# WangHelin1997/SSR-Speech

Hardware: AMD Instinct MI355X
Metric: codec-tokens/sec/GPU (AR decode) + RTF for 10 s TTS, English 830M (higher is better)
Workload: dtype f32; 1 GPU; English-830M-shape zero-shot TTS decode, cfg_stride=5, top_k=40/top_p=0.8 sampling, batch=1 (2 CFG rows) per GPU; L=130 phonemes, 160-frame prompt (demo/5895_34622_000026_000002.wav, first 3.2 s, wmencodec codes), context 304..324; utterances_per_gpu=1, rows=2, graph=True, steps_completed=25, pair_launches=True

## Files before the change

ssr-speech_amd/csrc/embed_sample.hip:

```cpp
#include <stdlib.h>
#include "common.h"

namespace {

__device__ __forceinline__ void embed_row(const ssrhip_embed_args& a, int r, int kind, int pos, const int* tok, int t0, int nt) {
  const int D = a.D;
  const float alpha = kind ? a.alpha_audio : a.alpha_text;
  for (int d = t0 * 4; d < D; d += nt * 4) {
    float4 e;
    if (kind == 0) {
      e = ld4(a.text_emb + (size_t)tok[0] * D + d);
    } else {
      float4 t[SSRHIP_MAX_CODEBOOKS];
#pragma unroll
      for (int k = 0; k < SSRHIP_MAX_CODEBOOKS; ++k)
        t[k] = (k < a.K) ? ld4(a.audio_emb + ((size_t)k * a.card + tok[k]) * D + d) : make_float4(0.f, 0.f, 0.f, 0.f);
      e = t[0];
#pragma unroll
      for (int k = 1; k < SSRHIP_MAX_CODEBOOKS; ++k) {
        if (k < a.K) { e.x += t[k].x; e.y += t[k].y; e.z += t[k].z; e.w += t[k].w; }
      }
    }
    const float4 p = ld4(a.pe + (size_t)pos * D + d);
    e.x = __fadd_rn(e.x, __fmul_rn(alpha, p.x));
    e.y = __fadd_rn(e.y, __fmul_rn(alpha, p.y));
    e.z = __fadd_rn(e.z, __fmul_rn(alpha, p.z));
    e.w = __fadd_rn(e.w, __fmul_rn(alpha, p.w));
    float* dst = a.out_tiled ? a.out + SSRHIP_TILED_P(r, d, D) : a.out + (size_t)r * D + d;
    *reinterpret_cast<float4*>(dst) = e;
  }
}

__global__ __launch_bounds__(256) void embed_kernel(const ssrhip_embed_args a) {
  const int r = blockIdx.x;
  embed_row(a, r, a.kind ? a.kind[r] : 1, a.pos[r], a.tok + (size_t)r * SSRHIP_MAX_CODEBOOKS, threadIdx.x, 256);
}

constexpr int MAXE = 9;
constexpr int WPC = 4;
constexpr int SAMPLE_THREADS = 64 * WPC * SSRHIP_MAX_CODEBOOKS;

#ifdef SSR_SAMPLE_PROFILE
__device__ unsigned long long g_sample_prof[16];
#define STAMP(i) do { if (threadIdx.x == 0) g_sample_prof[i] = __builtin_readcyclecounter(); } while (0)
#else
#define STAMP(i) do { } while (0)
#endif

__device__ __forceinline__ uint32_t okey(float f) {
  const uint32_t u = __float_as_uint(f);
  return (u & 0x80000000u) ? ~u : (u | 0x80000000u);
}

__device__ __forceinline__ uint32_t hash32(uint32_t x) {
  x ^= x >> 16; x *= 0x7feb352du; x ^= x >> 15; x *= 0x846ca68bu; x ^= x >> 16;
  return x;
}

template <class T>
__device__ __forceinline__ T suffix_excl(T v, int lane) {
  T inc = v;
#pragma unroll
  for (int o = 1; o < 64; o <<= 1) {
    const T t = __shfl_down(inc, o, 64);
    if (lane + o < 64) inc += t;
  }
  return inc - v;
}

struct SelShared {
  unsigned long long hist[SSRHIP_MAX_CODEBOOKS][WPC][256];
  unsigned long long carry[SSRHIP_MAX_CODEBOOKS];
  unsigned bin[SSRHIP_MAX_CODEBOOKS];
  int found[SSRHIP_MAX_CODEBOOKS];
  static constexpr int MAXC = 64;
  unsigned ckey[SSRHIP_MAX_CODEBOOKS][MAXC];
  unsigned long long cmass[SSRHIP_MAX_CODEBOOKS][MAXC];
  int ncand[SSRHIP_MAX_CODEBOOKS];
  unsigned result[SSRHIP_MAX_CODEBOOKS];
  int overflow;
};

template <int MODE>
__device__ __forceinline__ uint32_t radix_select(const uint32_t (&key)[MAXE], const float (&p)[MAXE], unsigned kk, float lim, bool active,
                                                 SelShared& sh, int k, int sub, int lane) {
  const float SC = 1099511627776.0f;
  const unsigned long long limfx = (unsigned long long)((double)lim * (double)SC);
  uint32_t prefix = 0, mask = 0;
  unsigned long long carry = (MODE == 0) ? (unsigned long long)kk : 0ull;
  bool keep_all = false;
  for (int pass = 0; pass < 4; ++pass) {
    const int shift = 24 - 8 * pass;
    unsigned long long* mine64 = sh.hist[k][sub];
    unsigned* mine32 = reinterpret_cast<unsigned*>(mine64);
    if (MODE == 0) { for (int j = lane; j < 256; j += 64) mine32[j] = 0u; }
    else { for (int j = lane; j < 256; j += 64) mine64[j] = 0ull; }
    __syncthreads();
    if (active && !keep_all) {
#pragma unroll
      for (int e = 0; e < MAXE; ++e) {
        const bool in = (MODE == 0) ? (key[e] != 0u) : (p[e] > 0.f);
        if (in && (key[e] & mask) == prefix) {
          if (MODE == 0) atomicAdd(&mine32[(key[e] >> shift) & 255u], 1u);
          else atomicAdd(&mine64[(key[e] >> shift) & 255u], (unsigned long long)(p[e] * SC));
        }
      }
    }
    __syncthreads();
    if (sub == 0 && active && !keep_all) {
      unsigned long long c[4] = {0ull, 0ull, 0ull, 0ull};
#pragma unroll
      for (int w = 0; w < WPC; ++w)
#pragma unroll
        for (int j = 0; j < 4; ++j)
          c[j] += (MODE == 0) ? (unsigned long long)reinterpret_cast<unsigned*>(sh.hist[k][w])[lane * 4 + j] : sh.hist[k][w][lane * 4 + j];
      const unsigned long long base = (MODE == 0) ? 0ull : carry;
      const unsigned long long a3 = base + suffix_excl<unsigned long long>(c[0] + c[1] + c[2] + c[3], lane);
      const unsigned long long a2 = a3 + c[3], a1 = a2 + c[2], a0 = a1 + c[1];
      int f = -1;
      unsigned long long above = 0;
      if (MODE == 0) {
        if (carry > a3 && carry <= a3 + c[3]) { f = 3; above = a3; }
        else if (carry > a2 && carry <= a2 + c[2]) { f = 2; above = a2; }
        else if (carry > a1 && carry <= a1 + c[1]) { f = 1; above = a1; }
        else if (carry > a0 && carry <= a0 + c[0]) { f = 0; above = a0; }
      } else {
        if (a3 <= limfx && limfx < a3 + c[3]) { f = 3; above = a3; }
        else if (a2 <= limfx && limfx < a2 + c[2]) { f = 2; above = a2; }
        else if (a1 <= limfx && limfx < a1 + c[1]) { f = 1; above = a1; }
        else if (a0 <= limfx && limfx < a0 + c[0]) { f = 0; above = a0; }
      }
      const unsigned long long bal = __ballot(f >= 0);
      if (lane == 0) sh.found[k] = bal ? 1 : 0;
      if (f >= 0) {
        sh.bin[k] = (unsigned)(lane * 4 + f);
        sh.carry[k] = (MODE == 0) ? (carry - above) : above;
      }
    }
    __syncthreads();
    if (active && !keep_all) {
      if (!sh.found[k]) keep_all = true;
      else {
        prefix |= sh.bin[k] << shift;
        mask |= 255u << shift;
        carry = sh.carry[k];
      }
    }
  }
  return keep_all ? 0u : prefix;
}

template <int MODE>
__device__ __forceinline__ uint32_t bin_select(const uint32_t (&key)[MAXE], const float (&p)[MAXE], const float (&l)[MAXE], float lo, float scale,
                                               unsigned kk, float lim, bool active, SelShared& sh, int k, int sub, int lane, int force_radix, bool& fallback) {
  const float SC = 1099511627776.0f;
  const unsigned long long limfx = (unsigned long long)((double)lim * (double)SC);
  unsigned long long* mine64 = sh.hist[k][sub];
  unsigned* mine32 = reinterpret_cast<unsigned*>(mine64);
  if (MODE == 0) { for (int j = lane; j < 256; j += 64) mine32[j] = 0u; }
  else { for (int j = lane; j < 256; j += 64) mine64[j] = 0ull; }
  if (threadIdx.x == 0) sh.overflow = force_radix;
  if (sub == 0 && lane == 0) { sh.ncand[k] = 0; sh.result[k] = 0u; }
  if (MODE == 0) STAMP(9);
  int vb[MAXE];
#pragma unroll
  for (int e = 0; e < MAXE; ++e) {
    const bool in = (MODE == 0) ? (key[e] != 0u) : (p[e] > 0.f);
    const int ob = min(254, max(1, 1 + (int)((l[e] - lo) * scale)));
    vb[e] = !in ? -1 : (l[e] >= 9000.f ? 255 : (l[e] <= -9000.f ? 0 : ob));
  }
  __syncthreads();
  if (MODE == 0) STAMP(10);
  if (active) {
#pragma unroll
    for (int e = 0; e < MAXE; ++e) {
      if (vb[e] >= 0) {
        if (MODE == 0) atomicAdd(&mine32[vb[e]], 1u);
        else atomicAdd(&mine64[vb[e]], (unsigned long long)(p[e] * SC));
      }
    }
  }
  __syncthreads();
  if (MODE == 0) STAMP(11);
  if (sub == 0 && active) {
    unsigned long long c[4] = {0ull, 0ull, 0ull, 0ull};
#pragma unroll
    for (int w = 0; w < WPC; ++w)
#pragma unroll
      for (int j = 0; j < 4; ++j)
        c[j] += (MODE == 0) ? (unsigned long long)reinterpret_cast<unsigned*>(sh.hist[k][w])[lane * 4 + j] : sh.hist[k][w][lane * 4 + j];
    const unsigned long long a3 = suffix_excl<unsigned long long>(c[0] + c[1] + c[2] + c[3], lane);
    const unsigned long long a2 = a3 + c[3], a1 = a2 + c[2], a0 = a1 + c[1];
    const unsigned long long need = (unsigned long long)kk;
    int f = -1;
    unsigned long long above = 0;
    if (MODE == 0) {
      if (need > a3 && need <= a3 + c[3]) { f = 3; above = a3; }
      else if (need > a2 && need <= a2 + c[2]) { f = 2; above = a2; }
      else if (need > a1 && need <= a1 + c[1]) { f = 1; above = a1; }
      else if (need > a0 && need <= a0 + c[0]) { f = 0; above = a0; }
    } else {
      if (a3 <= limfx && limfx < a3 + c[3]) { f = 3; above = a3; }
      else if (a2 <= limfx && limfx < a2 + c[2]) { f = 2; above = a2; }
      else if (a1 <= limfx && limfx < a1 + c[1]) { f = 1; above = a1; }
      else if (a0 <= limfx && limfx < a0 + c[0]) { f = 0; above = a0; }
    }
    const unsigned long long bal = __ballot(f >= 0);
    if (lane == 0) sh.found[k] = bal ? 1 : 0;
    if (f >= 0) {
      sh.bin[k] = (unsigned)(lane * 4 + f);
      sh.carry[k] = above;
    }
  }
  __syncthreads();
  if (MODE == 0) STAMP(12);
  const bool found = active && sh.found[k];
  const int bsel = found ? (int)sh.bin[k] : -2;
  const unsigned long long above_bins = found ? sh.carry[k] : 0ull;
  if (found) {
#pragma unroll
    for (int e = 0; e < MAXE; ++e) {
      if (vb[e] == bsel) {
        const int idx = atomicAdd(&sh.ncand[k], 1);
        if (idx < SelShared::MAXC) {
          sh.ckey[k][idx] = key[e];
          sh.cmass[k][idx] = (MODE == 0) ? 1ull : (unsigned long long)(p[e] * SC);
        }
      }
    }
  }
  __syncthreads();
  if (MODE == 0) STAMP(13);
  const int n = found ? sh.ncand[k] : 0;
  if (n > SelShared::MAXC) sh.overflow = 1;
  __syncthreads();
  if (MODE == 0) STAMP(14);
  fallback = sh.overflow != 0;
  if (!fallback) {
    unsigned todo = 0u;
#pragma unroll
    for (int e = 0; e < MAXE; ++e) todo |= (found && vb[e] == bsel) ? (1u << e) : 0u;
    while (__any(todo != 0u)) {
      uint32_t ke = 0u;
      bool mine = false;
      if (todo) {
        const int e0 = __builtin_ctz(todo);
        todo &= todo - 1u;
        mine = true;
#pragma unroll
        for (int e = 0; e < MAXE; ++e) ke = (e == e0) ? key[e] : ke;
      }
      unsigned long long A = above_bins, M = 0ull;
      for (int i = 0; i < n; ++i) {
        const unsigned ck = sh.ckey[k][i];
        const unsigned long long m = sh.cmass[k][i];
        A += (ck > ke) ? m : 0ull;
        M += (ck == ke) ? m : 0ull;
      }
      const bool hit = (MODE == 0) ? ((unsigned long long)kk > A && (unsigned long long)kk <= A + M) : (A <= limfx && limfx < A + M);
      if (mine && hit) sh.result[k] = ke;
    }
  }
  __syncthreads();
  if (MODE == 0) STAMP(15);
  return (found && !fallback) ? sh.result[k] : 0u;
}

__global__ __launch_bounds__(SAMPLE_THREADS) void sample_kernel(const ssrhip_sample_args a, const int force_radix) {
  __shared__ SelShared sel;
  __shared__ float sh_f[SSRHIP_MAX_CODEBOOKS][WPC];
  __shared__ float sh_g[SSRHIP_MAX_CODEBOOKS][WPC];
  __shared__ int sh_i[SSRHIP_MAX_CODEBOOKS][WPC];
  __shared__ int sh_sample[SSRHIP_MAX_CODEBOOKS];
  __shared__ int sh_argmax0;
  __shared__ int sh_next[SSRHIP_MAX_CODEBOOKS + 2];
  const int u = blockIdx.x;
  const ssrhip_sampler_cfg& c = a.cfg[u];
  ssrhip_sampler_state& st = a.state[u];
  if (st.done) return;
  const int lane = threadIdx.x & 63, wave = threadIdx.x >> 6;
  const int k = wave / WPC, sub = wave % WPC;
  const int K = a.K, card = a.card;
  const bool active = k < K;
  const int rows = c.use_cfg ? 2 : 1;
  const int row0 = u * rows;
  const int num_gen = st.num_gen, num_eog = st.num_eog, cfg_tag = st.num_cfg_tag;
  const int prev_token = st.prev_token, consec = st.consec_silence;
  const int step = st.n_steps;
  const int c_eos = c.eos, c_sos = c.sos, c_mts = c.mts, c_mts_end = c.mts + c.max_n_spans;
  const int c_empty = c.empty_token, c_eog = c.eog, c_topk = c.top_k, c_stoprep = c.stop_repetition;
  const float c_topp = c.top_p, c_temp = c.temperature, c_coef = c.cfg_coef, c_om = c.cfg_one_minus;
  const int c_maxsteps = c.max_steps, c_nsil = c.n_silence;
  const uint32_t c_seedlo = c.seed_lo, c_seedhi = c.seed_hi;
  const int c_usecfg = c.use_cfg, c_stride = c.cfg_stride, c_textlen = c.text_len, c_nspans = c.n_spans;
  const int st_audio_pos = st.audio_pos, st_span = st.span;
  int c_sil[SSRHIP_MAX_SILENCE];
#pragma unroll
  for (int j = 0; j < SSRHIP_MAX_SILENCE; ++j) c_sil[j] = c.silence[j];
  STAMP(0);

  const int kc = active ? k : 0;
  const float* lc = a.logits + ((size_t)row0 * K + kc) * card;
  const float* lu = lc + (size_t)K * card;
  const bool guided = c_usecfg && (cfg_tag == c_stride);
  bool penal = false;
  if (k == 0 && num_eog == 0 && c_stoprep > 0 && consec > c_stoprep) {
#pragma unroll
    for (int s = 0; s < SSRHIP_MAX_SILENCE; ++s) penal |= (s < c_nsil) && (c_sil[s] == prev_token);
  }
  const float npen = (float)(consec - (c_stoprep - 1));
  const bool force_empty = (num_gen < K - 1) && (k > num_gen);
  const bool cut_eog_empty = (num_eog > 0) && (k > num_eog);
  const bool cut_eog = (num_eog == 0) && (k >= 1);
  float l[MAXE], lun[MAXE];
#pragma unroll
  for (int e = 0; e < MAXE; ++e) {
    const int i = e * 256 + sub * 64 + lane;
    const int ic = (i < card) ? i : 0;
    l[e] = lc[ic];
    lun[e] = guided ? lu[ic] : 0.f;
  }
#pragma unroll
  for (int e = 0; e < MAXE; ++e) {
    const int i = e * 256 + sub * 64 + lane;
    float v = guided ? __fadd_rn(__fmul_rn(c_coef, l[e]), __fmul_rn(c_om, lun[e])) : l[e];
    const bool special = (i == c_eos) | (i == c_sos) | ((i >= c_mts) & (i < c_mts_end));
    v = special ? -10000.f : v;
    v = (force_empty & (i == c_empty)) ? 10000.f : v;
    v = (cut_eog_empty & ((i == c_eog) | (i == c_empty))) ? -10000.f : v;
    v = (cut_eog & (i == c_eog)) ? -10000.f : v;
    if (penal && i == prev_token) v = (v < 0.f) ? __fmul_rn(v, npen) : __fdiv_rn(v, npen);
    l[e] = (active && i < card) ? v : -INFINITY;
  }
  if (a.dbg_logits && active) {
    float* dbg = a.dbg_logits + ((size_t)u * K + k) * card;
#pragma unroll
    for (int e = 0; e < MAXE; ++e) {
      const int i = e * 256 + sub * 64 + lane;
      if (i < card) dbg[i] = l[e];
    }
  }
  STAMP(1);
  float mx = -INFINITY;
#pragma unroll
  for (int e = 0; e < MAXE; ++e) mx = fmaxf(mx, l[e]);
  mx = wave_max(mx);
  int am = 0x7fffffff;
#pragma unroll
  for (int e = 0; e < MAXE; ++e) if (l[e] == mx) am = min(am, e * 256 + sub * 64 + lane);
  am = wave_min_i(am);
  if (lane == 0 && active) { sh_f[k][sub] = mx; sh_i[k][sub] = am; }
  __syncthreads();
  if (active) {
    float m2 = sh_f[k][0];
    int a2 = sh_i[k][0];
#pragma unroll
    for (int w = 1; w < WPC; ++w)
      if (sh_f[k][w] > m2 || (sh_f[k][w] == m2 && sh_i[k][w] < a2)) { m2 = sh_f[k][w]; a2 = sh_i[k][w]; }
    mx = m2;
    am = a2;
  }
  __syncthreads();
  if (c_temp != 1.0f) {
#pragma unroll
    for (int e = 0; e < MAXE; ++e) l[e] = __fdiv_rn(l[e], c_temp);
    float m3 = -INFINITY;
#pragma unroll
    for (int e = 0; e < MAXE; ++e) m3 = fmaxf(m3, l[e]);
    m3 = wave_max(m3);
    if (lane == 0 && active) sh_f[k][sub] = m3;
    __syncthreads();
    if (active) mx = fmaxf(fmaxf(sh_f[k][0], sh_f[k][1]), fmaxf(sh_f[k][2], sh_f[k][3]));
    __syncthreads();
  }
  uint32_t key[MAXE];
#pragma unroll
  for (int e = 0; e < MAXE; ++e) key[e] = (active && (e * 256 + sub * 64 + lane) < card) ? okey(l[e]) : 0u;
  const uint32_t kmax = okey(mx);
  float vlo = INFINITY, vhi = -INFINITY;
#pragma unroll
  for (int e = 0; e < MAXE; ++e) {
    const bool ord = (key[e] != 0u) && (l[e] < 9000.f) && (l[e] > -9000.f);
    vlo = ord ? fminf(vlo, l[e]) : vlo;
    vhi = ord ? fmaxf(vhi, l[e]) : vhi;
  }
  vlo = -wave_max(-vlo);
  vhi = wave_max(vhi);
  if (lane == 0 && active) { sh_f[k][sub] = vlo; sh_g[k][sub] = vhi; }
  __syncthreads();
  if (active) {
    vlo = fminf(fminf(sh_f[k][0], sh_f[k][1]), fminf(sh_f[k][2], sh_f[k][3]));
    vhi = fmaxf(fmaxf(sh_g[k][0], sh_g[k][1]), fmaxf(sh_g[k][2], sh_g[k][3]));
  }
  __syncthreads();
  const float vscale = (vhi > vlo) ? 253.0f / (vhi - vlo) : 0.f;
  float p[MAXE];
#pragma unroll
  for (int e = 0; e < MAXE; ++e) p[e] = 0.f;
  STAMP(2);
  uint32_t thr = 0;
  if (c_topk > 0) {
    const int kk = min(max(c_topk, 1), card);
    if (kk == 1) thr = kmax;
    else if (kk < card) {
      bool fb;
      thr = bin_select<0>(key, p, l, vlo, vscale, (unsigned)kk, 0.f, active, sel, kc, sub, lane, force_radix, fb);
      if (fb) thr = radix_select<0>(key, p, (unsigned)kk, 0.f, active, sel, kc, sub, lane);
    }
  }
  STAMP(3);
  float Z = 0.f;
#pragma unroll
  for (int e = 0; e < MAXE; ++e) {
    p[e] = (key[e] != 0u && key[e] >= thr) ? __expf(l[e] - mx) : 0.f;
    Z += p[e];
  }
  Z = wave_sum(Z);
  if (lane == 0 && active) sh_f[k][sub] = Z;
  __syncthreads();
  if (active) Z = (sh_f[k][0] + sh_f[k][1]) + (sh_f[k][2] + sh_f[k][3]);
  __syncthreads();
  if (c_topp < 1.0f) {
    bool fb;
    uint32_t tp = bin_select<1>(key, p, l, vlo, vscale, 0u, c_topp * Z, active, sel, kc, sub, lane, force_radix, fb);
    if (fb) tp = radix_select<1>(key, p, 0u, c_topp * Z, active, sel, kc, sub, lane);
    if (tp > thr) {
      thr = tp;
#pragma unroll
      for (int e = 0; e < MAXE; ++e) p[e] = (key[e] >= thr) ? p[e] : 0.f;
    }
  }
  STAMP(4);
  {
    const float* nz = (a.noise && c.use_noise) ? a.noise + (((size_t)u * c_maxsteps + step) * K + kc) * card : nullptr;
    const uint32_t sd = hash32(c_seedlo + (uint32_t)step * 0x9E3779B1u) ^ hash32(c_seedhi + (uint32_t)kc * 0x85EBCA6Bu + 0x632BE5ABu);
    float best = -1.f;
    int bi = 0x7fffffff;
#pragma unroll
    for (int e = 0; e < MAXE; ++e) {
      const int i = e * 256 + sub * 64 + lane;
      float q;
      if (nz) q = nz[(key[e] != 0u) ? i : 0];
      else {
        const uint32_t hsh = hash32(sd + (uint32_t)i * 0x9E3779B1u);
        q = fmaxf(-__logf(((float)(hsh >> 8) + 1.0f) * (1.0f / 16777216.0f)), 1e-30f);
      }
      const float sc = (p[e] > 0.f) ? __fdividef(p[e], q) : -1.f;
      const bool better = sc > best;
      best = better ? sc : best;
      bi = better ? i : bi;
    }
    const float wb = wave_max(best);
    bi = (best == wb) ? bi : 0x7fffffff;
    bi = wave_min_i(bi);
    if (lane == 0 && active) { sh_f[k][sub] = wb; sh_i[k][sub] = bi; }
    __syncthreads();
    if (active && sub == 0 && lane == 0) {
      float b2 = sh_f[k][0];
      int i2 = sh_i[k][0];
#pragma unroll
      for (int w = 1; w < WPC; ++w)
        if (sh_f[k][w] > b2 || (sh_f[k][w] == b2 && sh_i[k][w] < i2)) { b2 = sh_f[k][w]; i2 = sh_i[k][w]; }
      sh_sample[k] = i2;
      if (k == 0) sh_argmax0 = am;
    }
  }
  STAMP(5);
  __syncthreads();
  STAMP(6);
  if (threadIdx.x == 0) {
    int s[SSRHIP_MAX_CODEBOOKS];
    for (int j = 0; j < K; ++j) s[j] = sh_sample[j];
    int ne_og = num_eog, cs = consec, pt = prev_token;
    if (num_eog > 0) {
      for (int j = 0; j < num_eog; ++j) s[j] = c_empty;
      s[num_eog] = c_eog;
      ne_og = num_eog + 1;
    } else {
      if (s[0] == c_eog || sh_argmax0 == c_eog || (st_audio_pos + 1) > c_textlen * 10) {
        s[0] = c_eog;
        ne_og = 1;
      }
      bool sil = false;
#pragma unroll
      for (int j = 0; j < SSRHIP_MAX_SILENCE; ++j) sil |= (j < c_nsil) && (c_sil[j] == s[0]);
      cs = (sil && s[0] == pt) ? cs + 1 : 0;
      pt = s[0];
    }
    if (c_usecfg) st.num_cfg_tag = (cfg_tag == c_stride) ? 1 : cfg_tag + 1;
    int* gen = a.generated + ((size_t)u * c_maxsteps + step) * K;
    for (int j = 0; j < K; ++j) gen[j] = s[j];
    st.n_steps = step + 1;
    st.num_gen = num_gen + 1;
    st.num_eog = ne_og;
    st.consec_silence = cs;
    st.prev_token = pt;
    bool done = false;
    int span = st_span;
    if (ne_og == K) {
      st.span_end[span] = step + 1;
      span += 1;
      st.span = span;
      if (span >= c_nspans) { st.done = 1; done = true; }
      else {
        st.num_gen = 0; st.num_eog = 0; st.num_cfg_tag = 1; st.prev_token = -1; st.consec_silence = 0;
        for (int j = 0; j < K; ++j) s[j] = c_mts + span;
      }
    }
    if (!done && step + 1 >= c_maxsteps) { st.done = 2; done = true; }
    sh_next[SSRHIP_MAX_CODEBOOKS + 1] = done ? 0 : 1;
    if (!done) {
      const int apos = st_audio_pos + 1;
      st.audio_pos = apos;
      sh_next[SSRHIP_MAX_CODEBOOKS] = apos;
      for (int j = 0; j < SSRHIP_MAX_CODEBOOKS; ++j) sh_next[j] = (j < K) ? s[j] : 0;
      for (int rr = 0; rr < rows; ++rr) {
        const int b = row0 + rr;
        for (int j = 0; j < SSRHIP_MAX_CODEBOOKS; ++j) a.next_tok[b * SSRHIP_MAX_CODEBOOKS + j] = (j < K) ? s[j] : 0;
        a.next_pos[b] = apos;
        const int kp = a.kv_pos[b] + 1;
        a.kv_pos[b] = kp;
        a.row_len[b] = kp + 1;
      }
    }
  }
  STAMP(7);
  if (a.embed.out) {
    __syncthreads();
    if (sh_next[SSRHIP_MAX_CODEBOOKS + 1]) {
      for (int rr = 0; rr < rows; ++rr) embed_row(a.embed, row0 + rr, 1, sh_next[SSRHIP_MAX_CODEBOOKS], sh_next, threadIdx.x, SAMPLE_THREADS);
    }
  }
  STAMP(8);
}

}

extern "C" int ssrhip_embed(const ssrhip_embed_args* a, ssrhip_stream_t stream) {
  SSR_REQUIRE(a && a->audio_emb && a->pe && a->tok && a->pos && a->out, "ssrhip_embed: null argument");
  SSR_REQUIRE(a->R > 0 && a->D % 4 == 0 && a->K >= 1 && a->K <= SSRHIP_MAX_CODEBOOKS, "ssrhip_embed: bad R/D/K");
  SSR_REQUIRE(!a->kind || a->text_emb, "ssrhip_embed: text rows need text_emb");
  hipLaunchKernelGGL(embed_kernel, dim3(a->R), dim3(256), 0, (hipStream_t)stream, *a);
  SSR_LAUNCH_CHECK();
  return 0;
}

extern "C" int ssrhip_sample(const ssrhip_sample_args* a, ssrhip_stream_t stream) {
  SSR_REQUIRE(a && a->logits && a->cfg && a->state && a->generated && a->next_tok && a->next_pos && a->kv_pos && a->row_len,
              "ssrhip_sample: null argument");
  SSR_REQUIRE(a->K >= 1 && a->K <= SSRHIP_MAX_CODEBOOKS, "ssrhip_sample: K=%d", a->K);
  SSR_REQUIRE(a->card > 0 && a->card <= 64 * WPC * MAXE, "ssrhip_sample: card=%d exceeds %d", a->card, 64 * WPC * MAXE);
  if (a->embed.out) SSR_REQUIRE(a->embed.audio_emb && a->embed.pe && a->embed.D % 4 == 0 && a->embed.K == a->K && a->embed.card == a->card,
                                "ssrhip_sample: fused embed needs audio_emb, pe, matching K/card");
  const char* e = getenv("SSRHIP_SAMPLE_RADIX");
  hipLaunchKernelGGL(sample_kernel, dim3(a->n_utt), dim3(SAMPLE_THREADS), 0, (hipStream_t)stream, *a, (e && atoi(e)) ? 1 : 0);
  SSR_LAUNCH_CHECK();
  return 0;
}
```

Baseline: 5388 codec-tokens/s.

## Sample from compacted top-k survivor list in one wave per codebook

After top-k thresholding, kept candidates are appended through shared-memory atomics to a per-codebook list of up to 64 entries. One wave per codebook then runs the top-p cutoff and the Gumbel-style draw over that list with cross-lane readlanes. This replaces the full-width top-p bin/radix select and the multi-wave argmax reduction. Overflow or the env flag falls back to the old path; the risks are atomic contention and the survivor path's ordering or rounding differing from the full-width one.

```diff
diff --git a/ssr-speech_amd/csrc/embed_sample.hip b/ssr-speech_amd/csrc/embed_sample.hip
--- a/ssr-speech_amd/csrc/embed_sample.hip
+++ b/ssr-speech_amd/csrc/embed_sample.hip
@@ -41,7 +41,7 @@
 constexpr int SAMPLE_THREADS = 64 * WPC * SSRHIP_MAX_CODEBOOKS;
 
 #ifdef SSR_SAMPLE_PROFILE
-__device__ unsigned long long g_sample_prof[16];
+__device__ unsigned long long g_sample_prof[24];
 #define STAMP(i) do { if (threadIdx.x == 0) g_sample_prof[i] = __builtin_readcyclecounter(); } while (0)
 #else
 #define STAMP(i) do { } while (0)
@@ -79,7 +79,13 @@
   int ncand[SSRHIP_MAX_CODEBOOKS];
   unsigned result[SSRHIP_MAX_CODEBOOKS];
   int overflow;
+  int cidx[SSRHIP_MAX_CODEBOOKS][MAXC];
+  float cp[SSRHIP_MAX_CODEBOOKS][MAXC];
+  int nsurv[SSRHIP_MAX_CODEBOOKS];
 };
+
+constexpr int SAMPLE_FORCE_RADIX = 1;
+constexpr int SAMPLE_FULL_WIDTH = 2;
 
 template <int MODE>
 __device__ __forceinline__ uint32_t radix_select(const uint32_t (&key)[MAXE], const float (&p)[MAXE], unsigned kk, float lim, bool active,
@@ -266,7 +272,55 @@
   return (found && !fallback) ? sh.result[k] : 0u;
 }
 
-__global__ __launch_bounds__(SAMPLE_THREADS) void sample_kernel(const ssrhip_sample_args a, const int force_radix) {
+__device__ __forceinline__ int survivor_draw(const ssrhip_sample_args& a, const SelShared& sh, int k, int lane, uint32_t thr, float top_p, float Z,
+                                             const float* nz, uint32_t sd) {
+  const int n = __builtin_amdgcn_readfirstlane(sh.nsurv[k]);
+  const bool have = lane < n;
+  const uint32_t ke = have ? sh.ckey[k][lane] : 0u;
+  const unsigned long long ms = have ? sh.cmass[k][lane] : 0ull;
+  const int i = have ? sh.cidx[k][lane] : 0;
+  const float pe = have ? sh.cp[k][lane] : 0.f;
+  if (top_p < 1.0f) {
+    const float SC = 1099511627776.0f;
+    const unsigned long long limfx = (unsigned long long)((double)(top_p * Z) * (double)SC);
+    const uint32_t mlo = (uint32_t)ms, mhi = (uint32_t)(ms >> 32);
+    unsigned long long Aj[4] = {0ull, 0ull, 0ull, 0ull}, Mj[4] = {0ull, 0ull, 0ull, 0ull};
+    for (int j = 0; j < n; j += 4) {
+#pragma unroll
+      for (int t = 0; t < 4; ++t) {
+        const uint32_t ck = (uint32_t)__builtin_amdgcn_readlane((int)ke, j + t);
+        const unsigned long long m = (unsigned long long)(uint32_t)__builtin_amdgcn_readlane((int)mlo, j + t) |
+                                     ((unsigned long long)(uint32_t)__builtin_amdgcn_readlane((int)mhi, j + t) << 32);
+        Aj[t] += (ck > ke) ? m : 0ull;
+        Mj[t] += (ck == ke) ? m : 0ull;
+      }
+    }
+    const unsigned long long A = (Aj[0] + Aj[1]) + (Aj[2] + Aj[3]), M = (Mj[0] + Mj[1]) + (Mj[2] + Mj[3]);
+    const bool hit = have && pe > 0.f && A <= limfx && limfx < A + M;
+    const unsigned long long bal = __ballot(hit);
+    const uint32_t tp = bal ? (uint32_t)__builtin_amdgcn_readlane((int)ke, __builtin_ctzll(bal)) : 0u;
+    thr = tp > thr ? tp : thr;
+  }
+  STAMP(4);
+  float sc = -1.f;
+  int bi = 0x7fffffff;
+  if (have && ke >= thr && pe > 0.f) {
+    float q;
+    if (nz) q = nz[i];
+    else {
+      const uint32_t hsh = hash32(sd + (uint32_t)i * 0x9E3779B1u);
+      q = fmaxf(-__logf(((float)(hsh >> 8) + 1.0f) * (1.0f / 16777216.0f)), 1e-30f);
+    }
+    const float s = __fdividef(pe, q);
+    if (s > -1.f) { sc = s; bi = i; }
+  }
+  const float wb = wave_max(sc);
+  bi = (sc == wb) ? bi : 0x7fffffff;
+  return wave_min_i(bi);
+}
+
+__global__ __launch_bounds__(SAMPLE_THREADS) void sample_kernel(const ssrhip_sample_args a, const int flags) {
+  const int force_radix = flags & SAMPLE_FORCE_RADIX;
   __shared__ SelShared sel;
   __shared__ float sh_f[SSRHIP_MAX_CODEBOOKS][WPC];
   __shared__ float sh_g[SSRHIP_MAX_CODEBOOKS][WPC];
@@ -278,6 +332,7 @@
   const ssrhip_sampler_cfg& c = a.cfg[u];
   ssrhip_sampler_state& st = a.state[u];
   if (st.done) return;
+  if (threadIdx.x < SSRHIP_MAX_CODEBOOKS) sel.nsurv[threadIdx.x] = 0;
   const int lane = threadIdx.x & 63, wave = threadIdx.x >> 6;
   const int k = wave / WPC, sub = wave % WPC;
   const int K = a.K, card = a.card;
@@ -409,60 +464,85 @@
     }
   }
   STAMP(3);
+  const bool want_list = (c_topk > 0) && !(flags & SAMPLE_FULL_WIDTH);
   float Z = 0.f;
 #pragma unroll
   for (int e = 0; e < MAXE; ++e) {
-    p[e] = (key[e] != 0u && key[e] >= thr) ? __expf(l[e] - mx) : 0.f;
+    const bool kept = key[e] != 0u && key[e] >= thr;
+    p[e] = kept ? __expf(l[e] - mx) : 0.f;
     Z += p[e];
+    if (want_list && kept) {
+      const int idx = atomicAdd(&sel.nsurv[kc], 1);
+      if (idx < SelShared::MAXC) {
+        sel.ckey[kc][idx] = key[e];
+        sel.cmass[kc][idx] = (p[e] > 0.f) ? (unsigned long long)(p[e] * 1099511627776.0f) : 0ull;
+        sel.cidx[kc][idx] = e * 256 + sub * 64 + lane;
+        sel.cp[kc][idx] = p[e];
+      }
+    }
   }
   Z = wave_sum(Z);
   if (lane == 0 && active) sh_f[k][sub] = Z;
   __syncthreads();
   if (active) Z = (sh_f[k][0] + sh_f[k][1]) + (sh_f[k][2] + sh_f[k][3]);
-  __syncthreads();
-  if (c_topp < 1.0f) {
-    bool fb;
-    uint32_t tp = bin_select<1>(key, p, l, vlo, vscale, 0u, c_topp * Z, active, sel, kc, sub, lane, force_radix, fb);
-    if (fb) tp = radix_select<1>(key, p, 0u, c_topp * Z, active, sel, kc, sub, lane);
-    if (tp > thr) {
-      thr = tp;
-#pragma unroll
-      for (int e = 0; e < MAXE; ++e) p[e] = (key[e] >= thr) ? p[e] : 0.f;
-    }
-  }
-  STAMP(4);
-  {
-    const float* nz = (a.noise && c.use_noise) ? a.noise + (((size_t)u * c_maxsteps + step) * K + kc) * card : nullptr;
-    const uint32_t sd = hash32(c_seedlo + (uint32_t)step * 0x9E3779B1u) ^ hash32(c_seedhi + (uint32_t)kc * 0x85EBCA6Bu + 0x632BE5ABu);
-    float best = -1.f;
-    int bi = 0x7fffffff;
-#pragma unroll
-    for (int e = 0; e < MAXE; ++e) {
-      const int i = e * 256 + sub * 64 + lane;
-      float q;
-      if (nz) q = nz[(key[e] != 0u) ? i : 0];
-      else {
-        const uint32_t hsh = hash32(sd + (uint32_t)i * 0x9E3779B1u);
-        q = fmaxf(-__logf(((float)(hsh >> 8) + 1.0f) * (1.0f / 16777216.0f)), 1e-30f);
-      }
-      const float sc = (p[e] > 0.f) ? __fdividef(p[e], q) : -1.f;
-      const bool better = sc > best;
-      best = better ? sc : best;
-      bi = better ? i : bi;
-    }
-    const float wb = wave_max(best);
-    bi = (best == wb) ? bi : 0x7fffffff;
-    bi = wave_min_i(bi);
-    if (lane == 0 && active) { sh_f[k][sub] = wb; sh_i[k][sub] = bi; }
+  bool survivors = want_list;
+  for (int j = 0; j < K; ++j) survivors = survivors && (sel.nsurv[j] <= SelShared::MAXC);
+  STAMP(16);
+  const float* nz = (a.noise && c.use_noise) ? a.noise + (((size_t)u * c_maxsteps + step) * K + kc) * card : nullptr;
+  const uint32_t sd = hash32(c_seedlo + (uint32_t)step * 0x9E3779B1u) ^ hash32(c_seedhi + (uint32_t)kc * 0x85EBCA6Bu + 0x632BE5ABu);
+  if (survivors) {
+    static_assert(SSRHIP_MAX_CODEBOOKS <= WPC, "one worker wave per codebook on a SIMD of its own");
+    if (active && sub == k) {
+      const int i2 = survivor_draw(a, sel, k, lane, thr, c_topp, Z, nz, sd);
+      if (lane == 0) {
+        sh_sample[k] = i2;
+        if (k == 0) sh_argmax0 = am;
+      }
+    }
+  } else {
     __syncthreads();
-    if (active && sub == 0 && lane == 0) {
-      float b2 = sh_f[k][0];
-      int i2 = sh_i[k][0];
-#pragma unroll
-      for (int w = 1; w < WPC; ++w)
-        if (sh_f[k][w] > b2 || (sh_f[k][w] == b2 && sh_i[k][w] < i2)) { b2 = sh_f[k][w]; i2 = sh_i[k][w]; }
-      sh_sample[k] = i2;
-      if (k == 0) sh_argmax0 = am;
+    if (c_topp < 1.0f) {
+      bool fb;
+      uint32_t tp = bin_select<1>(key, p, l, vlo, vscale, 0u, c_topp * Z, active, sel, kc, sub, lane, force_radix, fb);
+      if (fb) tp = radix_select<1>(key, p, 0u, c_topp * Z, active, sel, kc, sub, lane);
+      if (tp > thr) {
+        thr = tp;
+#pragma unroll
+        for (int e = 0; e < MAXE; ++e) p[e] = (key[e] >= thr) ? p[e] : 0.f;
+      }
+    }
+    STAMP(4);
+    {
+      float best = -1.f;
+      int bi = 0x7fffffff;
+#pragma unroll
+      for (int e = 0; e < MAXE; ++e) {
+        const int i = e * 256 + sub * 64 + lane;
+        float q;
+        if (nz) q = nz[(key[e] != 0u) ? i : 0];
+        else {
+          const uint32_t hsh = hash32(sd + (uint32_t)i * 0x9E3779B1u);
+          q = fmaxf(-__logf(((float)(hsh >> 8) + 1.0f) * (1.0f / 16777216.0f)), 1e-30f);
+        }
+        const float sc = (p[e] > 0.f) ? __fdividef(p[e], q) : -1.f;
+        const bool better = sc > best;
+        best = better ? sc : best;
+        bi = better ? i : bi;
+      }
+      const float wb = wave_max(best);
+      bi = (best == wb) ? bi : 0x7fffffff;
+      bi = wave_min_i(bi);
+      if (lane == 0 && active) { sh_f[k][sub] = wb; sh_i[k][sub] = bi; }
+      __syncthreads();
+      if (active && sub == 0 && lane == 0) {
+        float b2 = sh_f[k][0];
+        int i2 = sh_i[k][0];
+#pragma unroll
+        for (int w = 1; w < WPC; ++w)
+          if (sh_f[k][w] > b2 || (sh_f[k][w] == b2 && sh_i[k][w] < i2)) { b2 = sh_f[k][w]; i2 = sh_i[k][w]; }
+        sh_sample[k] = i2;
+        if (k == 0) sh_argmax0 = am;
+      }
     }
   }
   STAMP(5);
@@ -553,7 +633,9 @@
   if (a->embed.out) SSR_REQUIRE(a->embed.audio_emb && a->embed.pe && a->embed.D % 4 == 0 && a->embed.K == a->K && a->embed.card == a->card,
                                 "ssrhip_sample: fused embed needs audio_emb, pe, matching K/card");
   const char* e = getenv("SSRHIP_SAMPLE_RADIX");
-  hipLaunchKernelGGL(sample_kernel, dim3(a->n_utt), dim3(SAMPLE_THREADS), 0, (hipStream_t)stream, *a, (e && atoi(e)) ? 1 : 0);
+  const char* sv = getenv("SSRHIP_SAMPLE_SURVIVORS");
+  const int flags = ((e && atoi(e)) ? SAMPLE_FORCE_RADIX : 0) | ((sv && *sv && !atoi(sv)) ? SAMPLE_FULL_WIDTH : 0);
+  hipLaunchKernelGGL(sample_kernel, dim3(a->n_utt), dim3(SAMPLE_THREADS), 0, (hipStream_t)stream, *a, flags);
   SSR_LAUNCH_CHECK();
   return 0;
 }
```

After: 5402 codec-tokens/s, median of 2. About the same (+0.3%).
